# shamspias/fennec

Measured on AMD Instinct MI355X. Metric: megapixels/sec: 4K SSIMFast+GaussianBlur, higher is better.
Workload: dtype u8 (blur: exact int32 sums of 24-bit fixed-point weights on the i8 matrix pipe; fp64 SSIM)

## Files before the change

### fennec_amd/csrc/blur_mfma.hip

```cpp
#include <hip/hip_ext.h>

#include "common.hpp"
#include "devutil.hpp"

#include <algorithm>
#include <cmath>
#include <type_traits>
#include <vector>

namespace fnx {

typedef int v4i __attribute__((ext_vector_type(4)));

constexpr int MF_RMAX = 6;
constexpr int MF_P = 48;
constexpr int MF_WT = 64 * MF_P + 256;
constexpr int MF_SP = 352;
constexpr int MF_OP = 272;
constexpr int MF_SEG_SCORE = 272;
constexpr int MF_SEG_SCORE_WIDE = 544;

struct MfmaArgs {
    const uint8_t *src;
    const uint8_t *const *srcs;
    uint8_t *dst;
    uint8_t *const *dsts;
    int sstride, dstride, w, h;
    int tiles_x, tiles, seg;
    int radius;
    const uint32_t *tab;
    int seed_h, seed_v, thr;
    const int32_t *bx, *by;
    unsigned long long *slabs;
    int nbx, nby;
    int dbg;
};

__device__ __forceinline__ int mf_comb3(int hi, int mid, int lo)
{
    int t = hi * 256 + mid;
    asm volatile("" : "+v"(t));
    return t * 256 + lo;
}

__device__ __forceinline__ const double *mf_scalar_ptr(const double *p)
{
    const unsigned long long v = reinterpret_cast<unsigned long long>(p);
    const unsigned lo = __builtin_amdgcn_readfirstlane(static_cast<unsigned>(v)), hi = __builtin_amdgcn_readfirstlane(static_cast<unsigned>(v >> 32));
    return reinterpret_cast<const double *>((static_cast<unsigned long long>(hi) << 32) | lo);
}
typedef int mf_s16i __attribute__((ext_vector_type(16)));
__device__ __forceinline__ uint32_t mf_exact_u(const double *wd, const uint8_t *base, int step, int ring0, int mask)
{
    mf_s16i w0, w1;
    asm volatile("s_load_dwordx16 %0, %2, 0x0\n\ts_load_dwordx16 %1, %2, 0x40\n\ts_waitcnt lgkmcnt(0)" : "=&s"(w0), "=&s"(w1) : "s"(mf_scalar_ptr(wd)) : "memory");
    uint32_t v[13];
#pragma unroll
    for (int t = 0; t < 13; t++) v[t] = base[((ring0 + t) & mask) * step];
    double acc = 0;
#pragma unroll
    for (int t = 0; t < 13; t++) {
        const int lo = t < 8 ? w0[2 * (t & 7)] : w1[2 * (t & 7)], hi = t < 8 ? w0[2 * (t & 7) + 1] : w1[2 * (t & 7) + 1];
        acc = acc + u8_to_f64(v[t] ^ 0x80u) * __hiloint2double(hi, lo);
    }
    return clampF_dev(acc);
}

__device__ __forceinline__ void mf_box_add4(uint32_t *tbl, const u32x4 ro, uint32_t coln, const v4i cb)
{
#pragma unroll
    for (int k = 0; k < 4; k++)
        __hip_atomic_fetch_add(reinterpret_cast<uint32_t *>(reinterpret_cast<char *>(tbl) + ro[k] + coln), static_cast<uint32_t>(cb[k]),
                               __ATOMIC_RELAXED, __HIP_MEMORY_SCOPE_WORKGROUP);
}

template <bool SCORE, bool GUARD>
__global__ __launch_bounds__(256, GUARD ? 3 : 1) void blur_mfma_kernel(MfmaArgs a)
{
    constexpr int P = MF_P, WT = MF_WT, SP = MF_SP, OP = MF_OP;
    __shared__ __attribute__((aligned(16))) uint8_t s_t[4 * WT];
    __shared__ __attribute__((aligned(16))) uint8_t s_stage[2 * 16 * SP];
    __shared__ __attribute__((aligned(16))) uint8_t s_out[2 * 16 * OP];
    __shared__ __attribute__((aligned(16))) uint32_t s_rowh[SCORE ? MF_SEG_SCORE + 32 : 4];
    __shared__ __attribute__((aligned(16))) uint32_t s_rowv[SCORE ? MF_SEG_SCORE + 16 : 4];
    __shared__ uint32_t s_colbox[SCORE ? 64 : 1];
    extern __shared__ __attribute__((aligned(16))) uint32_t s_box[];

    const int tile = xcd_tile(blockIdx.x, a.tiles);
    if (tile < 0) return;
    const int z = blockIdx.y;
    const uint8_t *src = a.srcs ? a.srcs[z] : a.src;
    uint8_t *dst = a.dsts ? a.dsts[z] : a.dst;
    const int ty = tile / a.tiles_x, tx = tile - ty * a.tiles_x;
    const int x0 = tx * 64, y0 = ty * a.seg;
    const int tid = threadIdx.x, wave = tid >> 6, lane = tid & 63;
    const int r = lane & 15, g = lane >> 4;
    const int NJ = min(a.seg, ((a.h - y0 + 15) >> 4) << 4) >> 4;
    const int NI = NJ + 1;
    const bool xedge = x0 - 6 < 0 || x0 + 70 > a.w;

    const v4i *tbh = reinterpret_cast<const v4i *>(a.tab);
    const long *tbv = reinterpret_cast<const long *>(a.tab + 3 * 64 * 4);
    const v4i bh2 = tbh[lane], bh1 = tbh[64 + lane], bh0 = tbh[128 + lane];
    const long bv2 = tbv[lane], bv1 = tbv[64 + lane], bv0 = tbv[128 + lane];
    const bool alane = (r & 3) == 3;
    const int seed_hl = alane ? (1 << 23) + 128 : a.seed_h;
    const v4i sh = {seed_hl, seed_hl, seed_hl, seed_hl}, sv = {a.seed_v, a.seed_v, a.seed_v, a.seed_v};
    const v4i zero = {0, 0, 0, 0};
    const uint32_t sel01 = alane ? 0x0c0c0400u : 0x0c0c0703u, sel23 = alane ? 0x04000c0cu : 0x07030c0cu;

    uint8_t *tw = s_t + wave * WT;
    const int id1 = min(256 + tid, 16 * 19 - 1);
    const int srow0 = tid / 19, sch0 = tid - 19 * srow0, srow1 = id1 / 19, sch1 = id1 - 19 * srow1;
    const bool two = tid < 48;
    const int st_w0 = srow0 * SP + 16 * sch0, st_w1 = srow1 * SP + 16 * sch1;
    const int st_r = r * SP + 64 * wave + 16 * g;
    uint8_t *t_w = tw + r * P + 4 * g;
    const int m4 = r >> 2, mi = r & 3;
    const uint8_t *t_r = tw + (16 * m4 + mi) * P + 64 * m4 + 8 * g;
    const uint8_t *t_ro = tw + (16 * m4 + mi) * P + 64 * m4 + ((8 * g + 16) & 31);
    const uint8_t *t_ae = tw + (16 * g + 3) * P + 64 * g + r + 6;
    const uint8_t *t_ao = tw + (16 * g + 3) * P + 64 * g + ((r + 22) & 31);
    const int o_w = r * OP + 64 * wave + 16 * g;
    const int orow = tid >> 4, och = tid & 15;
    const int o_r = orow * OP + 16 * och;
    const int xo = x0 + 4 * och;

    v4i bbox = {0, 0, 0, 0}, sbox = {0, 0, 0, 0};
    uint32_t coln = 0;
    const int slabn = SCORE ? (a.nbx + 1) * (a.nby + 1) : 0;
    uint32_t *tbl_s = s_box, *tbl_b = s_box + 4 * slabn;
    auto score_setup = [&]() {
        if (!(a.dbg & 4)) for (int e = tid; e < 8 * slabn; e += 256) s_box[e] = 0;
        const int rowbytes = 16 * (a.nbx + 1);
        const int b0y = a.by[y0];
        for (int u = tid; u < 16 * NI; u += 256) {
            const int t = u - 6;
            const int v = (t >= 0 && t < a.seg && y0 + t < a.h) ? a.by[y0 + t] : -1;
            s_rowh[u] = rowbytes * ((v >= 0 && b0y >= 0) ? v - b0y : a.nby);
        }
        for (int t = tid; t < 16 * NJ; t += 256) {
            const int v = (t < a.seg && y0 + t < a.h) ? a.by[y0 + t] : -1;
            s_rowv[t] = rowbytes * ((v >= 0 && b0y >= 0) ? v - b0y : a.nby);
        }
        if (tid < 64) {
            const int b0x = a.bx[x0], v = x0 + tid < a.w ? a.bx[x0 + tid] : -1;
            s_colbox[tid] = (v >= 0 && b0x >= 0) ? v - b0x : 255u;
        }
        __syncthreads();
        uint32_t first = 255u;
        for (int i = 0; i < 16; i++) first = min(first, s_colbox[16 * wave + i]);
        const int slot = r / 3, ch = r - 3 * slot;
        int cnt = 0;
        for (int i = 0; i < 16; i++) cnt += (r < 15 && s_colbox[16 * wave + i] == first + slot) ? 1 : 0;
#pragma unroll
        for (int e = 0; e < 4; e++) {
            const bool in = r < 15 && first != 255u && s_colbox[16 * wave + 4 * g + e] == first + slot;
            bbox[e] = in ? (1 << (8 * ch)) : 0;
        }
        const int seed = 128 * cnt;
        sbox = (v4i){seed, seed, seed, seed};
        const uint32_t bc = (r < 15 && first != 255u && cnt > 0) ? first + slot : static_cast<uint32_t>(a.nbx);
        coln = 16u * bc + 4u * (r < 15 ? ch : 3);
    };

    const double *wd = reinterpret_cast<const double *>(a.tab + 3 * 64 * 4 + 3 * 64 * 2);

    auto stage_write = [&](const u32x4 (&d)[2], int buf) {
        uint8_t *sb = s_stage + buf * 16 * SP;
        *reinterpret_cast<u32x4 *>(sb + st_w0) = d[0] ^ 0x80808080u;
        if (two) *reinterpret_cast<u32x4 *>(sb + st_w1) = d[1] ^ 0x80808080u;
    };
    auto hset = [&](int s, int buf, int slot) {
        const uint8_t *sbuf = s_stage + buf * 16 * SP;
        const uint8_t *sb = sbuf + st_r;
        if constexpr (!GUARD && !SCORE) {
#pragma unroll
            for (int hf = 0; hf < 2; hf++) {
                v4i c2[2], c1[2], c0[2];
#pragma unroll
                for (int q2 = 0; q2 < 2; q2++) {
                    const v4i A = *reinterpret_cast<const v4i *>(sb + 16 * (2 * hf + q2));
                    c2[q2] = __builtin_amdgcn_mfma_i32_16x16x64_i8(A, bh2, zero, 0, 0, 0);
                    c1[q2] = __builtin_amdgcn_mfma_i32_16x16x64_i8(A, bh1, zero, 0, 0, 0);
                    c0[q2] = __builtin_amdgcn_mfma_i32_16x16x64_i8(A, bh0, sh, 0, 0, 0);
                }
#pragma unroll
                for (int q2 = 0; q2 < 2; q2++) {
                    const int qq = 2 * hf + q2;
                    v4i u;
#pragma unroll
                    for (int k = 0; k < 4; k++) u[k] = mf_comb3(c2[q2][k], c1[q2][k], c0[q2][k]);
                    const uint32_t t01 = __builtin_amdgcn_perm((uint32_t)u[1], (uint32_t)u[0], sel01);
                    const uint32_t t23 = __builtin_amdgcn_perm((uint32_t)u[3], (uint32_t)u[2], sel23);
                    *reinterpret_cast<uint32_t *>(t_w + (16 * qq) * P + 64 * qq + 16 * slot) = t01 | t23;
                }
                __builtin_amdgcn_sched_barrier(0);
            }
            return;
        }
        v4i c2[4], c1[4], c0[4];
#pragma unroll
        for (int qq = 0; qq < 4; qq++) {
            const v4i A = *reinterpret_cast<const v4i *>(sb + 16 * qq);
            c2[qq] = __builtin_amdgcn_mfma_i32_16x16x64_i8(A, bh2, zero, 0, 0, 0);
            c1[qq] = __builtin_amdgcn_mfma_i32_16x16x64_i8(A, bh1, zero, 0, 0, 0);
            c0[qq] = __builtin_amdgcn_mfma_i32_16x16x64_i8(A, bh0, sh, 0, 0, 0);
        }
        if constexpr (SCORE) {
            const u32x2 lo = *reinterpret_cast<const u32x2 *>(sb + 24), hi = *reinterpret_cast<const u32x2 *>(sb + 32);
            const v4i A = {(int)lo.x, (int)lo.y, (int)hi.x, (int)hi.y};
            const v4i cb = __builtin_amdgcn_mfma_i32_16x16x64_i8(A, bbox, sbox, 0, 0, 0);
            const u32x4 ro = *reinterpret_cast<const u32x4 *>(s_rowh + 16 * s + 4 * g);
            if (!(a.dbg & 1)) mf_box_add4(tbl_s, ro, coln, cb);
        }
        v4i u[4];
#pragma unroll
        for (int qq = 0; qq < 4; qq++)
#pragma unroll
            for (int k = 0; k < 4; k++) u[qq][k] = mf_comb3(c2[qq][k], c1[qq][k], c0[qq][k]);
#pragma unroll
        for (int qq = 0; qq < 4; qq++) {
            const uint32_t t01 = __builtin_amdgcn_perm((uint32_t)u[qq][1], (uint32_t)u[qq][0], sel01);
            const uint32_t t23 = __builtin_amdgcn_perm((uint32_t)u[qq][3], (uint32_t)u[qq][2], sel23);
            *reinterpret_cast<uint32_t *>(t_w + (16 * qq) * P + 64 * qq + 16 * slot) = t01 | t23;
        }
        if constexpr (GUARD) {
            uint32_t m[4];
#pragma unroll
            for (int qq = 0; qq < 4; qq++) {
                const uint32_t f0 = static_cast<uint32_t>(u[qq][0]) & 0x00ffffffu, f1 = static_cast<uint32_t>(u[qq][1]) & 0x00ffffffu;
                const uint32_t f2 = static_cast<uint32_t>(u[qq][2]) & 0x00ffffffu, f3 = static_cast<uint32_t>(u[qq][3]) & 0x00ffffffu;
                m[qq] = min(min(min(f0, f1), f2), f3);
            }
            const uint32_t mm = min(min(min(m[0], m[1]), m[2]), m[3]);
            if (__builtin_amdgcn_ballot_w64(mm < static_cast<uint32_t>(a.thr))) {
                uint32_t fl = 0;
#pragma unroll
                for (int qq = 0; qq < 4; qq++)
#pragma unroll
                    for (int k = 0; k < 4; k++) fl |= ((static_cast<uint32_t>(u[qq][k]) & 0x00ffffffu) < static_cast<uint32_t>(a.thr) ? 1u : 0u) << (4 * qq + k);
                unsigned long long todo = __builtin_amdgcn_ballot_w64(fl != 0);
                while (todo) {
                    const int L = __builtin_ctzll(todo);
                    todo &= todo - 1;
                    uint32_t flL = __builtin_amdgcn_readlane(fl, L);
                    const int rL = L & 15, gL = L >> 4;
                    while (flL) {
                        const int b = __builtin_ctz(flL), qq = b >> 2, k = b & 3;
                        flL &= flL - 1;
                        const uint32_t e = mf_exact_u(wd, sbuf + (4 * gL + k) * SP + 4 * (16 * wave + 4 * qq + (rL >> 2)) + (rL & 3), 4, 0, 0xffff) ^ 0x80u;
                        if (lane == L) *(t_w + (16 * qq) * P + 64 * qq + 16 * slot + k) = static_cast<uint8_t>(e);
                    }
                }
            }
        }
    };
    auto vset = [&](int j, int buf, auto oddt) {
        constexpr bool ODD = decltype(oddt)::value;
        long A[4];
        uint32_t al[4];
#pragma unroll
        for (int q = 0; q < 4; q++) A[q] = *reinterpret_cast<const long *>((ODD ? t_ro : t_r) + (4 * q) * P);
#pragma unroll
        for (int q = 0; q < 4; q++) al[q] = *((ODD ? t_ao : t_ae) + (4 * q) * P);
        int u[4][3];
        if constexpr (!GUARD && !SCORE) {
#pragma unroll
            for (int hf = 0; hf < 2; hf++) {
                v4i c2[2], c1[2], c0[2];
#pragma unroll
                for (int q2 = 0; q2 < 2; q2++) {
                    c2[q2] = __builtin_amdgcn_mfma_i32_16x16x32_i8(A[2 * hf + q2], bv2, zero, 0, 0, 0);
                    c1[q2] = __builtin_amdgcn_mfma_i32_16x16x32_i8(A[2 * hf + q2], bv1, zero, 0, 0, 0);
                    c0[q2] = __builtin_amdgcn_mfma_i32_16x16x32_i8(A[2 * hf + q2], bv0, sv, 0, 0, 0);
                }
#pragma unroll
                for (int q2 = 0; q2 < 2; q2++)
#pragma unroll
                    for (int i = 0; i < 3; i++) u[2 * hf + q2][i] = mf_comb3(c2[q2][i], c1[q2][i], c0[q2][i]);
                __builtin_amdgcn_sched_barrier(0);
            }
        } else {
            v4i c2[4], c1[4], c0[4];
#pragma unroll
            for (int q = 0; q < 4; q++) {
                c2[q] = __builtin_amdgcn_mfma_i32_16x16x32_i8(A[q], bv2, zero, 0, 0, 0);
                c1[q] = __builtin_amdgcn_mfma_i32_16x16x32_i8(A[q], bv1, zero, 0, 0, 0);
                c0[q] = __builtin_amdgcn_mfma_i32_16x16x32_i8(A[q], bv0, sv, 0, 0, 0);
            }
#pragma unroll
            for (int q = 0; q < 4; q++)
#pragma unroll
                for (int i = 0; i < 3; i++) u[q][i] = mf_comb3(c2[q][i], c1[q][i], c0[q][i]);
        }
        u32x4 o;
#pragma unroll
        for (int q = 0; q < 4; q++) {
            const uint32_t t01 = __builtin_amdgcn_perm((uint32_t)u[q][1], (uint32_t)u[q][0], 0x0c0c0703u);
            const uint32_t t23 = __builtin_amdgcn_perm(al[q], (uint32_t)u[q][2], 0x04030c0cu);
            o[q] = t01 | t23;
        }
        uint8_t *op = s_out + buf * 16 * OP + o_w;
        *reinterpret_cast<u32x4 *>(op) = o;
        if constexpr (GUARD) {
            uint32_t m[4];
#pragma unroll
            for (int q = 0; q < 4; q++)
                m[q] = min(min(static_cast<uint32_t>(u[q][0]) & 0x00ffffffu, static_cast<uint32_t>(u[q][1]) & 0x00ffffffu), static_cast<uint32_t>(u[q][2]) & 0x00ffffffu);
            const uint32_t mm = min(min(min(m[0], m[1]), m[2]), m[3]);
            if (__builtin_amdgcn_ballot_w64(mm < static_cast<uint32_t>(a.thr))) {
                uint32_t fl = 0;
#pragma unroll
                for (int q = 0; q < 4; q++)
#pragma unroll
                    for (int i = 0; i < 3; i++) fl |= ((static_cast<uint32_t>(u[q][i]) & 0x00ffffffu) < static_cast<uint32_t>(a.thr) ? 1u : 0u) << (4 * q + i);
                unsigned long long todo = __builtin_amdgcn_ballot_w64(fl != 0);
                while (todo) {
                    const int L = __builtin_ctzll(todo);
                    todo &= todo - 1;
                    uint32_t flL = __builtin_amdgcn_readlane(fl, L);
                    const int rL = L & 15, gL = L >> 4;
                    while (flL) {
                        const int b = __builtin_ctz(flL), q = b >> 2, i = b & 3;
                        flL &= flL - 1;
                        const uint32_t e = mf_exact_u(wd, tw + (16 * gL + 4 * q + i) * P + 64 * gL, 1, (ODD ? 16 : 0) + rL, 31);
                        if (lane == L) op[4 * q + i] = static_cast<uint8_t>(e);
                    }
                }
                if constexpr (SCORE) o = *reinterpret_cast<const u32x4 *>(op);
            }
        }
        if constexpr (SCORE) {
            const u32x4 os = o ^ 0x80808080u;
            const v4i A = {(int)os[0], (int)os[1], (int)os[2], (int)os[3]};
            const v4i cb = __builtin_amdgcn_mfma_i32_16x16x64_i8(A, bbox, sbox, 0, 0, 0);
            const u32x4 ro = *reinterpret_cast<const u32x4 *>(s_rowv + 16 * j + 4 * g);
            if (!(a.dbg & 1)) mf_box_add4(tbl_b, ro, coln, cb);
        }
    };

    auto march = [&](auto xedget) {
        constexpr bool XEDGE = decltype(xedget)::value;
        auto hload = [&](int i, u32x4 (&d)[2]) {
            const int ys = y0 - 6 + 16 * i;
            if constexpr (!XEDGE) {
                const uint8_t *sb = src + 4 * static_cast<ptrdiff_t>(x0 - 6);
                const int ya = clampi(ys + srow0, 0, a.h - 1), yb = clampi(ys + srow1, 0, a.h - 1);
                d[0] = *(g_u32x4 *)(sb + static_cast<ptrdiff_t>(ya) * a.sstride + 16 * sch0);
                d[1] = *(g_u32x4 *)(sb + static_cast<ptrdiff_t>(yb) * a.sstride + 16 * sch1);
            } else {
    #pragma unroll
                for (int k = 0; k < 2; k++) {
                    if (k == 1 && !two) break;
                    const int y = clampi(ys + (k ? srow1 : srow0), 0, a.h - 1);
                    const uint8_t *rowp = src + static_cast<size_t>(y) * a.sstride;
                    const int xc = x0 - 6 + 4 * (k ? sch1 : sch0);
    #pragma unroll
                    for (int e = 0; e < 4; e++) d[k][e] = ld_px(rowp, clampi(xc + e, 0, a.w - 1));
                }
            }
        };
        auto out_store = [&](int j, int buf) {
            const u32x4 o = *reinterpret_cast<const u32x4 *>(s_out + buf * 16 * OP + o_r);
            const int y = y0 + 16 * j + orow;
            if (y < a.h) {
                uint8_t *dp = dst + static_cast<size_t>(y) * a.dstride + 4 * static_cast<size_t>(xo);
                if (!XEDGE || xo + 3 < a.w) *(g_u32x4w *)(dp) = o;
                else {
    #pragma unroll
                    for (int e = 0; e < 4; e++) if (xo + e < a.w) *(g_u32w *)(dp + 4 * e) = o[e];
                }
            }
        };
        u32x4 ra[2], rb[2];
        hload(0, ra);
        __builtin_amdgcn_sched_barrier(0);
        hload(min(1, NI - 1), rb);
        __builtin_amdgcn_sched_barrier(0);
        if constexpr (SCORE) score_setup();
        auto step = [&](int s, u32x4 (&d)[2], auto oddv) {
            constexpr int par = decltype(oddv)::value ? 0 : 1;
            if (s < NI) stage_write(d, par);
            if (XEDGE) { if (s + 2 < NI) hload(s + 2, d); } else hload(min(s + 2, NI - 1), d);
            if (s >= 3 && s - 3 < NJ) out_store(s - 3, par);
            __syncthreads();
            if (s < NI) hset(s, par, par);
            if (s >= 1 && s - 1 < NJ) vset(s - 1, par, oddv);
        };
    #pragma unroll 1
        for (int s = 0; s < NJ + 3; s += 2) {
            step(s, ra, std::true_type{});
            step(s + 1, rb, std::false_type{});
        }

    };
    if (xedge) march(std::true_type{}); else march(std::false_type{});

    if (SCORE && !(a.dbg & 2)) {
        __syncthreads();
        unsigned long long *slab = a.slabs + (static_cast<size_t>(z) * a.tiles + tile) * 2 * slabn;
        for (int e = tid; e < 2 * slabn; e += 256) {
            const u32x4 v = *reinterpret_cast<const u32x4 *>(s_box + 4 * e);
            slab[e] = static_cast<unsigned long long>(v.x | (v.y << 16)) | (static_cast<unsigned long long>(v.z) << 32);
        }
    }
}

template <int NKH> struct MfWide {
    static constexpr int NKV = NKH <= 4 ? 1 : (NKH <= 7 ? 2 : 3);
    static constexpr int RFH = 8 * NKH - 2, RFV = 32 * NKV - 8;
    static constexpr int RF = RFH < RFV ? RFH : RFV;
    static constexpr int NC = 16 + RF / 2;
    static constexpr int NL = (16 * NC + 255) / 256;
    static constexpr int SP = 16 * NC + 48;
    static constexpr int NT = 2 * RF + 1;
    static constexpr int NS = 4 * NKV;
    static constexpr int RING = 16 * NS;
    static constexpr int P = RING + 16;
    static constexpr int WT = 64 * P + 256;
};

template <int NT>
__device__ __noinline__ uint32_t mf_exact_h_n(const uint8_t *p, const double *wd)
{
    double acc = 0;
#pragma unroll 15
    for (int t = 0; t < NT; t++) acc = acc + u8_to_f64(p[4 * t] ^ 0x80u) * wd[t];
    return clampF_dev(acc);
}
template <int NT, int RING = 64>
__device__ __noinline__ uint32_t mf_exact_v_n(const uint8_t *p, int ring0, const double *wd)
{
    double acc = 0;
#pragma unroll 15
    for (int t = 0; t < NT; t++) acc = acc + u8_to_f64(p[static_cast<unsigned>(ring0 + t) % static_cast<unsigned>(RING)] ^ 0x80u) * wd[t];
    return clampF_dev(acc);
}

template <int NT>
__device__ __forceinline__ uint32_t mf_exact_u_n(const double *wd, const uint8_t *base, int step, int ring0, int mask)
{
    double acc = 0;
#pragma unroll
    for (int t0 = 0; t0 < NT; t0 += 8) {
        mf_s16i w;
        asm volatile("s_load_dwordx16 %0, %1, %2\n\ts_waitcnt lgkmcnt(0)" : "=&s"(w) : "s"(mf_scalar_ptr(wd)), "n"(8 * t0) : "memory");
        uint32_t v[8];
#pragma unroll
        for (int t = 0; t < 8; t++) v[t] = base[((ring0 + t0 + min(t, NT - 1 - t0)) & mask) * step];
#pragma unroll
        for (int t = 0; t < 8; t++)
            if (t0 + t < NT) acc = acc + u8_to_f64(v[t] ^ 0x80u) * __hiloint2double(w[2 * t + 1], w[2 * t]);
    }
    return clampF_dev(acc);
}

template <int NKH, bool GUARD, bool SCORE = false>
__global__ __launch_bounds__(256, MfWide<NKH>::NKV == 3 ? 1 : 2) void blur_mfma_wide_kernel(MfmaArgs a)
{
    using C = MfWide<NKH>;
    constexpr int RF = C::RF, NC = C::NC, SP = C::SP, P = C::P, WT = C::WT, OP = MF_OP, NT = C::NT;
    constexpr int NKV = C::NKV, NS = C::NS, RING = C::RING, NL = C::NL;
    static_assert(!SCORE || (4 * RF) % 8 == 0, "the source-side A operand is read as two 8-byte halves");
    static_assert(!SCORE || NKV == 1, "the one-pass form is NKH = 2's");
    __shared__ __attribute__((aligned(16))) uint8_t s_t[4 * WT];
    __shared__ __attribute__((aligned(16))) uint8_t s_stage[2 * 16 * SP];
    __shared__ __attribute__((aligned(16))) uint8_t s_out[2 * 16 * OP];
    __shared__ __attribute__((aligned(16))) uint32_t s_rowh[SCORE ? MF_SEG_SCORE_WIDE + 48 : 4];
    __shared__ __attribute__((aligned(16))) uint32_t s_rowv[SCORE ? MF_SEG_SCORE_WIDE + 16 : 4];
    __shared__ uint32_t s_colbox[SCORE ? 64 : 1];
    extern __shared__ __attribute__((aligned(16))) uint32_t s_box[];

    const int tile = xcd_tile(blockIdx.x, a.tiles);
    if (tile < 0) return;
    const int z = blockIdx.y;
    const uint8_t *src = a.srcs ? a.srcs[z] : a.src;
    uint8_t *dst = a.dsts ? a.dsts[z] : a.dst;
    const int ty = tile / a.tiles_x, tx = tile - ty * a.tiles_x;
    const int x0 = tx * 64, y0 = ty * a.seg;
    const int tid = threadIdx.x, wave = tid >> 6, lane = tid & 63;
    const int r = lane & 15, g = lane >> 4;
    const int NJ = min(a.seg, ((a.h - y0 + 15) >> 4) << 4) >> 4;
    const int NI = NJ + NS - 1;
    const bool xedge = x0 - RF < 0 || x0 + 64 + RF > a.w;

    const v4i *tbh = reinterpret_cast<const v4i *>(a.tab);
    v4i bh[NKH][3];
#pragma unroll
    for (int kk = 0; kk < NKH; kk++)
#pragma unroll
        for (int l = 0; l < 3; l++) bh[kk][l] = tbh[(3 * kk + l) * 64 + lane];
    const v4i *tbv = tbh + 3 * NKH * 64;
    v4i bv[NKV][3];
#pragma unroll
    for (int c = 0; c < NKV; c++)
#pragma unroll
        for (int l = 0; l < 3; l++) bv[c][l] = tbv[(3 * c + l) * 64 + lane];
    const double *wd = reinterpret_cast<const double *>(tbv + 3 * NKV * 64);
    const bool alane = (r & 3) == 3;
    const int seed_hl = alane ? (1 << 23) + 128 : a.seed_h;
    const v4i sh = {seed_hl, seed_hl, seed_hl, seed_hl}, sv = {a.seed_v, a.seed_v, a.seed_v, a.seed_v};
    const v4i zero = {0, 0, 0, 0};
    const uint32_t sel01 = alane ? 0x0c0c0400u : 0x0c0c0703u, sel23 = alane ? 0x04000c0cu : 0x07030c0cu;

    uint8_t *tw = s_t + wave * WT;
    int srow[NL], sch[NL], st_w[NL];
    bool have[NL];
#pragma unroll
    for (int k = 0; k < NL; k++) {
        const int id = min(256 * k + tid, 16 * NC - 1);
        srow[k] = id / NC; sch[k] = id - NC * srow[k];
        st_w[k] = srow[k] * SP + 16 * sch[k];
        have[k] = 256 * k + tid < 16 * NC;
    }
    const int st_r = r * SP + 64 * wave + 16 * g;
    uint8_t *t_w = tw + r * P + 4 * g;
    const int m4 = r >> 2, mi = r & 3;
    const uint8_t *t_r = tw + (16 * m4 + mi) * P + 64 * m4;
    const uint8_t *t_a = tw + (16 * g + 3) * P + 64 * g;
    const int o_w = r * OP + 64 * wave + 16 * g;
    const int orow = tid >> 4, och = tid & 15;
    const int o_r = orow * OP + 16 * och;
    const int xo = x0 + 4 * och;

    v4i bbox = {0, 0, 0, 0}, sbox = {0, 0, 0, 0};
    uint32_t coln = 0;
    const int slabn = SCORE ? (a.nbx + 1) * (a.nby + 1) : 0;
    uint32_t *tbl_s = s_box, *tbl_b = s_box + 4 * slabn;
    auto score_setup = [&]() {
        for (int e = tid; e < 8 * slabn; e += 256) s_box[e] = 0;
        const int rowbytes = 16 * (a.nbx + 1);
        const int b0y = a.by[y0];
        for (int u = tid; u < 16 * NI; u += 256) {
            const int t = u - RF;
            const int v = (t >= 0 && t < a.seg && y0 + t < a.h) ? a.by[y0 + t] : -1;
            s_rowh[u] = rowbytes * ((v >= 0 && b0y >= 0) ? v - b0y : a.nby);
        }
        for (int t = tid; t < 16 * NJ; t += 256) {
            const int v = (t < a.seg && y0 + t < a.h) ? a.by[y0 + t] : -1;
            s_rowv[t] = rowbytes * ((v >= 0 && b0y >= 0) ? v - b0y : a.nby);
        }
        if (tid < 64) {
            const int b0x = a.bx[x0], v = x0 + tid < a.w ? a.bx[x0 + tid] : -1;
            s_colbox[tid] = (v >= 0 && b0x >= 0) ? v - b0x : 255u;
        }
        __syncthreads();
        uint32_t first = 255u;
        for (int i = 0; i < 16; i++) first = min(first, s_colbox[16 * wave + i]);
        const int slot = r / 3, ch = r - 3 * slot;
        int cnt = 0;
        for (int i = 0; i < 16; i++) cnt += (r < 15 && s_colbox[16 * wave + i] == first + slot) ? 1 : 0;
#pragma unroll
        for (int e = 0; e < 4; e++) {
            const bool in = r < 15 && first != 255u && s_colbox[16 * wave + 4 * g + e] == first + slot;
            bbox[e] = in ? (1 << (8 * ch)) : 0;
        }
        const int seed = 128 * cnt;
        sbox = (v4i){seed, seed, seed, seed};
        const uint32_t bc = (r < 15 && first != 255u && cnt > 0) ? first + slot : static_cast<uint32_t>(a.nbx);
        coln = 16u * bc + 4u * (r < 15 ? ch : 3);
    };

    auto stage_write = [&](const u32x4 (&d)[NL], int buf) {
        uint8_t *sb = s_stage + buf * 16 * SP;
        *reinterpret_cast<u32x4 *>(sb + st_w[0]) = d[0] ^ 0x80808080u;
#pragma unroll
        for (int k = 1; k < NL; k++)
            if (have[k]) *reinterpret_cast<u32x4 *>(sb + st_w[k]) = d[k] ^ 0x80808080u;
    };
    auto hset = [&](int s, int buf, int slot) {
        const uint8_t *sbuf = s_stage + buf * 16 * SP;
        const uint8_t *sb = sbuf + st_r;
        v4i c2[4], c1[4], c0[4];
#pragma unroll
        for (int qq = 0; qq < 4; qq++) { c2[qq] = zero; c1[qq] = zero; c0[qq] = sh; }
        if constexpr (SCORE) {
            const u32x2 lo = *reinterpret_cast<const u32x2 *>(sb + 4 * RF), hi = *reinterpret_cast<const u32x2 *>(sb + 4 * RF + 8);
            const v4i A = {(int)lo.x, (int)lo.y, (int)hi.x, (int)hi.y};
            const v4i cb = __builtin_amdgcn_mfma_i32_16x16x64_i8(A, bbox, sbox, 0, 0, 0);
            const u32x4 ro = *reinterpret_cast<const u32x4 *>(s_rowh + 16 * s + 4 * g);
#pragma unroll
            for (int k = 0; k < 4; k++)
                __hip_atomic_fetch_add(reinterpret_cast<uint32_t *>(reinterpret_cast<char *>(tbl_s) + ro[k] + coln), static_cast<uint32_t>(cb[k]),
                                       __ATOMIC_RELAXED, __HIP_MEMORY_SCOPE_WORKGROUP);
        }
#pragma unroll
        for (int kk = 0; kk < NKH; kk++)
#pragma unroll
            for (int qq = 0; qq < 4; qq++) {
                const v4i A = *reinterpret_cast<const v4i *>(sb + 16 * qq + 64 * kk);
                c2[qq] = __builtin_amdgcn_mfma_i32_16x16x64_i8(A, bh[kk][0], c2[qq], 0, 0, 0);
                c1[qq] = __builtin_amdgcn_mfma_i32_16x16x64_i8(A, bh[kk][1], c1[qq], 0, 0, 0);
                c0[qq] = __builtin_amdgcn_mfma_i32_16x16x64_i8(A, bh[kk][2], c0[qq], 0, 0, 0);
            }
        v4i u[4];
#pragma unroll
        for (int qq = 0; qq < 4; qq++)
#pragma unroll
            for (int k = 0; k < 4; k++) u[qq][k] = mf_comb3(c2[qq][k], c1[qq][k], c0[qq][k]);
#pragma unroll
        for (int qq = 0; qq < 4; qq++) {
            const uint32_t t01 = __builtin_amdgcn_perm((uint32_t)u[qq][1], (uint32_t)u[qq][0], sel01);
            const uint32_t t23 = __builtin_amdgcn_perm((uint32_t)u[qq][3], (uint32_t)u[qq][2], sel23);
            *reinterpret_cast<uint32_t *>(t_w + (16 * qq) * P + 64 * qq + 16 * slot) = t01 | t23;
        }
        if constexpr (GUARD) {
            uint32_t m[4];
#pragma unroll
            for (int qq = 0; qq < 4; qq++) {
                const uint32_t f0 = static_cast<uint32_t>(u[qq][0]) & 0x00ffffffu, f1 = static_cast<uint32_t>(u[qq][1]) & 0x00ffffffu;
                const uint32_t f2 = static_cast<uint32_t>(u[qq][2]) & 0x00ffffffu, f3 = static_cast<uint32_t>(u[qq][3]) & 0x00ffffffu;
                m[qq] = min(min(min(f0, f1), f2), f3);
            }
            const uint32_t mm = min(min(min(m[0], m[1]), m[2]), m[3]);
            if (__builtin_amdgcn_ballot_w64(mm < static_cast<uint32_t>(a.thr))) {
                uint32_t fl = 0;
#pragma unroll
                for (int qq = 0; qq < 4; qq++)
#pragma unroll
                    for (int k = 0; k < 4; k++) fl |= ((static_cast<uint32_t>(u[qq][k]) & 0x00ffffffu) < static_cast<uint32_t>(a.thr) ? 1u : 0u) << (4 * qq + k);
                if constexpr (NKH > 2) {
                    while (fl) {
                        const int b = __builtin_ctz(fl), qq = b >> 2, k = b & 3;
                        fl &= fl - 1;
                        const uint32_t e = mf_exact_h_n<NT>(sbuf + (4 * g + k) * SP + 4 * (16 * wave + 4 * qq + (r >> 2)) + (r & 3), wd) ^ 0x80u;
                        *(t_w + (16 * qq) * P + 64 * qq + 16 * slot + k) = static_cast<uint8_t>(e);
                    }
                }
                unsigned long long todo = NKH > 2 ? 0ull : __builtin_amdgcn_ballot_w64(fl != 0);
                while (todo) {
                    const int L = __builtin_ctzll(todo);
                    todo &= todo - 1;
                    uint32_t flL = __builtin_amdgcn_readlane(fl, L);
                    const int rL = L & 15, gL = L >> 4;
                    while (flL) {
                        const int b = __builtin_ctz(flL), qq = b >> 2, k = b & 3;
                        flL &= flL - 1;
                        const uint32_t e = mf_exact_u_n<NT>(wd, sbuf + (4 * gL + k) * SP + 4 * (16 * wave + 4 * qq + (rL >> 2)) + (rL & 3), 4, 0, 0xffff) ^ 0x80u;
                        if (lane == L) *(t_w + (16 * qq) * P + 64 * qq + 16 * slot + k) = static_cast<uint8_t>(e);
                    }
                }
            }
        }
    };
    auto vset = [&](int j, int buf) {
        uint32_t al[4];
        const int jm = static_cast<int>(static_cast<unsigned>(j) % static_cast<unsigned>(NS));
        const int ra_ = static_cast<int>(static_cast<unsigned>(16 * jm + r + RF) % static_cast<unsigned>(RING));
#pragma unroll
        for (int q = 0; q < 4; q++) al[q] = *(t_a + (4 * q) * P + ra_);
        v4i c2[4], c1[4], c0[4];
#pragma unroll
        for (int q = 0; q < 4; q++) { c2[q] = zero; c1[q] = zero; c0[q] = sv; }
#pragma unroll
        for (int c = 0; c < NKV; c++) {
            const int ro = 16 * static_cast<int>(static_cast<unsigned>(jm + 4 * c + g) % static_cast<unsigned>(NS));
            v4i A[4];
#pragma unroll
            for (int q = 0; q < 4; q++) A[q] = *reinterpret_cast<const v4i *>(t_r + (4 * q) * P + ro);
#pragma unroll
            for (int q = 0; q < 4; q++) {
                c2[q] = __builtin_amdgcn_mfma_i32_16x16x64_i8(A[q], bv[c][0], c2[q], 0, 0, 0);
                c1[q] = __builtin_amdgcn_mfma_i32_16x16x64_i8(A[q], bv[c][1], c1[q], 0, 0, 0);
                c0[q] = __builtin_amdgcn_mfma_i32_16x16x64_i8(A[q], bv[c][2], c0[q], 0, 0, 0);
            }
        }
        int u[4][3];
#pragma unroll
        for (int q = 0; q < 4; q++)
#pragma unroll
            for (int i = 0; i < 3; i++) u[q][i] = mf_comb3(c2[q][i], c1[q][i], c0[q][i]);
        u32x4 o;
#pragma unroll
        for (int q = 0; q < 4; q++) {
            const uint32_t t01 = __builtin_amdgcn_perm((uint32_t)u[q][1], (uint32_t)u[q][0], 0x0c0c0703u);
            const uint32_t t23 = __builtin_amdgcn_perm(al[q], (uint32_t)u[q][2], 0x04030c0cu);
            o[q] = t01 | t23;
        }
        uint8_t *op = s_out + buf * 16 * OP + o_w;
        *reinterpret_cast<u32x4 *>(op) = o;
        if constexpr (GUARD) {
            uint32_t m[4];
#pragma unroll
            for (int q = 0; q < 4; q++)
                m[q] = min(min(static_cast<uint32_t>(u[q][0]) & 0x00ffffffu, static_cast<uint32_t>(u[q][1]) & 0x00ffffffu), static_cast<uint32_t>(u[q][2]) & 0x00ffffffu);
            const uint32_t mm = min(min(min(m[0], m[1]), m[2]), m[3]);
            if (__builtin_amdgcn_ballot_w64(mm < static_cast<uint32_t>(a.thr))) {
                uint32_t fl = 0;
#pragma unroll
                for (int q = 0; q < 4; q++)
#pragma unroll
                    for (int i = 0; i < 3; i++) fl |= ((static_cast<uint32_t>(u[q][i]) & 0x00ffffffu) < static_cast<uint32_t>(a.thr) ? 1u : 0u) << (4 * q + i);
                if constexpr (NKH > 2) {
                    while (fl) {
                        const int b = __builtin_ctz(fl), q = b >> 2, i = b & 3;
                        fl &= fl - 1;
                        op[4 * q + i] = static_cast<uint8_t>(mf_exact_v_n<NT, RING>(tw + (16 * g + 4 * q + i) * P + 64 * g, 16 * jm + r, wd));
                    }
                }
                unsigned long long todo = NKH > 2 ? 0ull : __builtin_amdgcn_ballot_w64(fl != 0);
                while (todo) {
// ... 399 lines not shown
```

Before: 395,600.

## Software-pipeline MFMA chains and defer LDS box atomics in the SCORE blur path

In the SCORE variant, the horizontal and vertical MFMA passes are rewritten to interleave the next quad's MFMAs with the combine and pack ALU work of the current quad, using sched barriers to fix the order. The LDS atomic box-sum adds from the horizontal pass are deferred into the vertical pass so they overlap MFMA latency. Atomic addresses are precomputed as LDS offsets. The march loop is split into prologue, steady-state and epilogue phases so the steady phase drops its bounds checks, and the debug flags become compile-time zero outside develop builds. The risks are higher register pressure and rigid scheduling from the many sched barriers.

```diff
diff --git a/fennec_amd/csrc/blur_mfma.hip b/fennec_amd/csrc/blur_mfma.hip
--- a/fennec_amd/csrc/blur_mfma.hip
+++ b/fennec_amd/csrc/blur_mfma.hip
@@ -36,11 +36,15 @@
     int dbg;
 };
 
-__device__ __forceinline__ int mf_comb3(int hi, int mid, int lo)
+__device__ __forceinline__ int mf_comb_hi(int hi, int mid)
 {
     int t = hi * 256 + mid;
     asm volatile("" : "+v"(t));
-    return t * 256 + lo;
+    return t;
+}
+__device__ __forceinline__ int mf_comb3(int hi, int mid, int lo)
+{
+    return mf_comb_hi(hi, mid) * 256 + lo;
 }
 
 __device__ __forceinline__ const double *mf_scalar_ptr(const double *p)
@@ -66,12 +70,21 @@
     return clampF_dev(acc);
 }
 
-__device__ __forceinline__ void mf_box_add4(uint32_t *tbl, const u32x4 ro, uint32_t coln, const v4i cb)
+typedef __attribute__((address_space(3))) uint32_t mf_lds_u32;
+__device__ __forceinline__ void mf_box_addr4(uint32_t (&ad)[4], uint32_t *tbl, const u32x4 ro, uint32_t coln)
+{
+    const uint32_t base = static_cast<uint32_t>(reinterpret_cast<uintptr_t>((mf_lds_u32 *)tbl)) + coln;
+#pragma unroll
+    for (int k = 0; k < 4; k++) {
+        ad[k] = ro[k] + base;
+        asm volatile("" : "+v"(ad[k]));
+    }
+}
+__device__ __forceinline__ void mf_box_add4(const uint32_t (&ad)[4], const v4i cb)
 {
 #pragma unroll
     for (int k = 0; k < 4; k++)
-        __hip_atomic_fetch_add(reinterpret_cast<uint32_t *>(reinterpret_cast<char *>(tbl) + ro[k] + coln), static_cast<uint32_t>(cb[k]),
-                               __ATOMIC_RELAXED, __HIP_MEMORY_SCOPE_WORKGROUP);
+        __hip_atomic_fetch_add((mf_lds_u32 *)static_cast<uintptr_t>(ad[k]), static_cast<uint32_t>(cb[k]), __ATOMIC_RELAXED, __HIP_MEMORY_SCOPE_WORKGROUP);
 }
 
 template <bool SCORE, bool GUARD>
@@ -130,8 +143,13 @@
     uint32_t coln = 0;
     const int slabn = SCORE ? (a.nbx + 1) * (a.nby + 1) : 0;
     uint32_t *tbl_s = s_box, *tbl_b = s_box + 4 * slabn;
+#ifdef FNX_DEVELOP
+    const int dbg = a.dbg;
+#else
+    constexpr int dbg = 0;
+#endif
     auto score_setup = [&]() {
-        if (!(a.dbg & 4)) for (int e = tid; e < 8 * slabn; e += 256) s_box[e] = 0;
+        if (!(dbg & 4)) for (int e = tid; e < 8 * slabn; e += 256) s_box[e] = 0;
         const int rowbytes = 16 * (a.nbx + 1);
         const int b0y = a.by[y0];
         for (int u = tid; u < 16 * NI; u += 256) {
@@ -171,7 +189,10 @@
         *reinterpret_cast<u32x4 *>(sb + st_w0) = d[0] ^ 0x80808080u;
         if (two) *reinterpret_cast<u32x4 *>(sb + st_w1) = d[1] ^ 0x80808080u;
     };
-    auto hset = [&](int s, int buf, int slot) {
+    v4i h_cb = zero;
+    uint32_t h_ad[4] = {0, 0, 0, 0};
+    auto hset = [&](int s, int buf, int slot, auto defert) {
+        constexpr bool DEFER = decltype(defert)::value;
         const uint8_t *sbuf = s_stage + buf * 16 * SP;
         const uint8_t *sb = sbuf + st_r;
         if constexpr (!GUARD && !SCORE) {
@@ -199,31 +220,62 @@
             }
             return;
         }
-        v4i c2[4], c1[4], c0[4];
-#pragma unroll
-        for (int qq = 0; qq < 4; qq++) {
-            const v4i A = *reinterpret_cast<const v4i *>(sb + 16 * qq);
-            c2[qq] = __builtin_amdgcn_mfma_i32_16x16x64_i8(A, bh2, zero, 0, 0, 0);
-            c1[qq] = __builtin_amdgcn_mfma_i32_16x16x64_i8(A, bh1, zero, 0, 0, 0);
-            c0[qq] = __builtin_amdgcn_mfma_i32_16x16x64_i8(A, bh0, sh, 0, 0, 0);
-        }
+        v4i u[4];
         if constexpr (SCORE) {
+            __builtin_amdgcn_sched_barrier(0);
+            v4i A[4];
+#pragma unroll
+            for (int qq = 0; qq < 4; qq++) A[qq] = *reinterpret_cast<const v4i *>(sb + 16 * qq);
             const u32x2 lo = *reinterpret_cast<const u32x2 *>(sb + 24), hi = *reinterpret_cast<const u32x2 *>(sb + 32);
-            const v4i A = {(int)lo.x, (int)lo.y, (int)hi.x, (int)hi.y};
-            const v4i cb = __builtin_amdgcn_mfma_i32_16x16x64_i8(A, bbox, sbox, 0, 0, 0);
+            const v4i As = {(int)lo.x, (int)lo.y, (int)hi.x, (int)hi.y};
             const u32x4 ro = *reinterpret_cast<const u32x4 *>(s_rowh + 16 * s + 4 * g);
-            if (!(a.dbg & 1)) mf_box_add4(tbl_s, ro, coln, cb);
-        }
-        v4i u[4];
-#pragma unroll
-        for (int qq = 0; qq < 4; qq++)
-#pragma unroll
-            for (int k = 0; k < 4; k++) u[qq][k] = mf_comb3(c2[qq][k], c1[qq][k], c0[qq][k]);
-#pragma unroll
-        for (int qq = 0; qq < 4; qq++) {
-            const uint32_t t01 = __builtin_amdgcn_perm((uint32_t)u[qq][1], (uint32_t)u[qq][0], sel01);
-            const uint32_t t23 = __builtin_amdgcn_perm((uint32_t)u[qq][3], (uint32_t)u[qq][2], sel23);
-            *reinterpret_cast<uint32_t *>(t_w + (16 * qq) * P + 64 * qq + 16 * slot) = t01 | t23;
+            v4i c2 = __builtin_amdgcn_mfma_i32_16x16x64_i8(A[0], bh2, zero, 0, 0, 0);
+            v4i c1 = __builtin_amdgcn_mfma_i32_16x16x64_i8(A[0], bh1, zero, 0, 0, 0);
+            v4i c0 = __builtin_amdgcn_mfma_i32_16x16x64_i8(A[0], bh0, sh, 0, 0, 0);
+            __builtin_amdgcn_sched_barrier(0);
+            mf_box_addr4(h_ad, tbl_s, ro, coln);
+            __builtin_amdgcn_sched_barrier(0);
+#pragma unroll
+            for (int qq = 0; qq < 4; qq++) {
+                v4i n2 = zero, n1 = zero, n0 = zero;
+                if (qq < 3) n2 = __builtin_amdgcn_mfma_i32_16x16x64_i8(A[qq + 1], bh2, zero, 0, 0, 0);
+                else h_cb = __builtin_amdgcn_mfma_i32_16x16x64_i8(As, bbox, sbox, 0, 0, 0);
+                __builtin_amdgcn_sched_barrier(0);
+                int t[4];
+#pragma unroll
+                for (int k = 0; k < 4; k++) t[k] = mf_comb_hi(c2[k], c1[k]);
+                __builtin_amdgcn_sched_barrier(0);
+                if (qq < 3) { n1 = __builtin_amdgcn_mfma_i32_16x16x64_i8(A[qq + 1], bh1, zero, 0, 0, 0); __builtin_amdgcn_sched_barrier(0); }
+#pragma unroll
+                for (int k = 0; k < 4; k++) u[qq][k] = t[k] * 256 + c0[k];
+                __builtin_amdgcn_sched_barrier(0);
+                if (qq < 3) { n0 = __builtin_amdgcn_mfma_i32_16x16x64_i8(A[qq + 1], bh0, sh, 0, 0, 0); __builtin_amdgcn_sched_barrier(0); }
+                const uint32_t t01 = __builtin_amdgcn_perm((uint32_t)u[qq][1], (uint32_t)u[qq][0], sel01);
+                const uint32_t t23 = __builtin_amdgcn_perm((uint32_t)u[qq][3], (uint32_t)u[qq][2], sel23);
+                *reinterpret_cast<uint32_t *>(t_w + (16 * qq) * P + 64 * qq + 16 * slot) = t01 | t23;
+                __builtin_amdgcn_sched_barrier(0);
+                c2 = n2; c1 = n1; c0 = n0;
+            }
+            if constexpr (!DEFER) { if (!(dbg & 1)) mf_box_add4(h_ad, h_cb); }
+        } else {
+            v4i c2[4], c1[4], c0[4];
+#pragma unroll
+            for (int qq = 0; qq < 4; qq++) {
+                const v4i A = *reinterpret_cast<const v4i *>(sb + 16 * qq);
+                c2[qq] = __builtin_amdgcn_mfma_i32_16x16x64_i8(A, bh2, zero, 0, 0, 0);
+                c1[qq] = __builtin_amdgcn_mfma_i32_16x16x64_i8(A, bh1, zero, 0, 0, 0);
+                c0[qq] = __builtin_amdgcn_mfma_i32_16x16x64_i8(A, bh0, sh, 0, 0, 0);
+            }
+#pragma unroll
+            for (int qq = 0; qq < 4; qq++)
+#pragma unroll
+                for (int k = 0; k < 4; k++) u[qq][k] = mf_comb3(c2[qq][k], c1[qq][k], c0[qq][k]);
+#pragma unroll
+            for (int qq = 0; qq < 4; qq++) {
+                const uint32_t t01 = __builtin_amdgcn_perm((uint32_t)u[qq][1], (uint32_t)u[qq][0], sel01);
+                const uint32_t t23 = __builtin_amdgcn_perm((uint32_t)u[qq][3], (uint32_t)u[qq][2], sel23);
+                *reinterpret_cast<uint32_t *>(t_w + (16 * qq) * P + 64 * qq + 16 * slot) = t01 | t23;
+            }
         }
         if constexpr (GUARD) {
             uint32_t m[4];
@@ -256,8 +308,9 @@
             }
         }
     };
-    auto vset = [&](int j, int buf, auto oddt) {
+    auto vset = [&](int j, int buf, auto oddt, auto defert) {
         constexpr bool ODD = decltype(oddt)::value;
+        constexpr bool DEFER = decltype(defert)::value;
         long A[4];
         uint32_t al[4];
 #pragma unroll
@@ -265,6 +318,16 @@
 #pragma unroll
         for (int q = 0; q < 4; q++) al[q] = *((ODD ? t_ao : t_ae) + (4 * q) * P);
         int u[4][3];
+        u32x4 o;
+        u32x4 v_ro = {0, 0, 0, 0};
+        uint32_t v_ad[4] = {0, 0, 0, 0};
+        if constexpr (SCORE) v_ro = *reinterpret_cast<const u32x4 *>(s_rowv + 16 * j + 4 * g);
+        auto pack = [&](int q) {
+            const uint32_t t01 = __builtin_amdgcn_perm((uint32_t)u[q][1], (uint32_t)u[q][0], 0x0c0c0703u);
+            const uint32_t t23 = __builtin_amdgcn_perm(al[q], (uint32_t)u[q][2], 0x04030c0cu);
+            o[q] = t01 | t23;
+        };
+        if constexpr (SCORE) __builtin_amdgcn_sched_barrier(0);
         if constexpr (!GUARD && !SCORE) {
 #pragma unroll
             for (int hf = 0; hf < 2; hf++) {
@@ -281,6 +344,34 @@
                     for (int i = 0; i < 3; i++) u[2 * hf + q2][i] = mf_comb3(c2[q2][i], c1[q2][i], c0[q2][i]);
                 __builtin_amdgcn_sched_barrier(0);
             }
+        } else if constexpr (SCORE) {
+            v4i c2 = __builtin_amdgcn_mfma_i32_16x16x32_i8(A[0], bv2, zero, 0, 0, 0);
+            if constexpr (DEFER) { if (!(dbg & 1)) mf_box_add4(h_ad, h_cb); }
+            v4i c1 = __builtin_amdgcn_mfma_i32_16x16x32_i8(A[0], bv1, zero, 0, 0, 0);
+            v4i c0 = __builtin_amdgcn_mfma_i32_16x16x32_i8(A[0], bv0, sv, 0, 0, 0);
+            __builtin_amdgcn_sched_barrier(0);
+            mf_box_addr4(v_ad, tbl_b, v_ro, coln);
+            __builtin_amdgcn_sched_barrier(0);
+#pragma unroll
+            for (int q = 0; q < 4; q++) {
+                v4i n2 = zero, n1 = zero, n0 = zero;
+                if (q < 3) { n2 = __builtin_amdgcn_mfma_i32_16x16x32_i8(A[q + 1], bv2, zero, 0, 0, 0); __builtin_amdgcn_sched_barrier(0); }
+                int t[3];
+#pragma unroll
+                for (int i = 0; i < 3; i++) t[i] = mf_comb_hi(c2[i], c1[i]);
+                asm volatile("" : : "v"(c2), "v"(c1));
+                __builtin_amdgcn_sched_barrier(0);
+                if (q < 3) { n1 = __builtin_amdgcn_mfma_i32_16x16x32_i8(A[q + 1], bv1, zero, 0, 0, 0); __builtin_amdgcn_sched_barrier(0); }
+#pragma unroll
+                for (int i = 0; i < 3; i++) { u[q][i] = t[i] * 256 + c0[i]; asm volatile("" : "+v"(u[q][i])); }
+                asm volatile("" : : "v"(c0));
+                __builtin_amdgcn_sched_barrier(0);
+                if (q < 3) { n0 = __builtin_amdgcn_mfma_i32_16x16x32_i8(A[q + 1], bv0, sv, 0, 0, 0); __builtin_amdgcn_sched_barrier(0); }
+                pack(q);
+                asm volatile("" : "+v"(o[q]));
+                __builtin_amdgcn_sched_barrier(0);
+                c2 = n2; c1 = n1; c0 = n0;
+            }
         } else {
             v4i c2[4], c1[4], c0[4];
 #pragma unroll
@@ -294,15 +385,13 @@
 #pragma unroll
                 for (int i = 0; i < 3; i++) u[q][i] = mf_comb3(c2[q][i], c1[q][i], c0[q][i]);
         }
-        u32x4 o;
-#pragma unroll
-        for (int q = 0; q < 4; q++) {
-            const uint32_t t01 = __builtin_amdgcn_perm((uint32_t)u[q][1], (uint32_t)u[q][0], 0x0c0c0703u);
-            const uint32_t t23 = __builtin_amdgcn_perm(al[q], (uint32_t)u[q][2], 0x04030c0cu);
-            o[q] = t01 | t23;
+        if constexpr (!SCORE) {
+#pragma unroll
+            for (int q = 0; q < 4; q++) pack(q);
         }
         uint8_t *op = s_out + buf * 16 * OP + o_w;
         *reinterpret_cast<u32x4 *>(op) = o;
+        if constexpr (SCORE) __builtin_amdgcn_sched_barrier(0);
         if constexpr (GUARD) {
             uint32_t m[4];
 #pragma unroll
@@ -335,8 +424,7 @@
             const u32x4 os = o ^ 0x80808080u;
             const v4i A = {(int)os[0], (int)os[1], (int)os[2], (int)os[3]};
             const v4i cb = __builtin_amdgcn_mfma_i32_16x16x64_i8(A, bbox, sbox, 0, 0, 0);
-            const u32x4 ro = *reinterpret_cast<const u32x4 *>(s_rowv + 16 * j + 4 * g);
-            if (!(a.dbg & 1)) mf_box_add4(tbl_b, ro, coln, cb);
+            if (!(dbg & 1)) mf_box_add4(v_ad, cb);
         }
     };
 
@@ -379,25 +467,44 @@
         hload(min(1, NI - 1), rb);
         __builtin_amdgcn_sched_barrier(0);
         if constexpr (SCORE) score_setup();
-        auto step = [&](int s, u32x4 (&d)[2], auto oddv) {
+        auto step = [&](int s, u32x4 (&d)[2], auto oddv, auto steadyt) {
             constexpr int par = decltype(oddv)::value ? 0 : 1;
-            if (s < NI) stage_write(d, par);
-            if (XEDGE) { if (s + 2 < NI) hload(s + 2, d); } else hload(min(s + 2, NI - 1), d);
-            if (s >= 3 && s - 3 < NJ) out_store(s - 3, par);
+            constexpr bool STEADY = decltype(steadyt)::value;
+            if (STEADY || s < NI) stage_write(d, par);
+            if (XEDGE && !STEADY) { if (s + 2 < NI) hload(s + 2, d); } else hload(min(s + 2, NI - 1), d);
+            if (STEADY || (s >= 3 && s - 3 < NJ)) out_store(s - 3, par);
             __syncthreads();
-            if (s < NI) hset(s, par, par);
-            if (s >= 1 && s - 1 < NJ) vset(s - 1, par, oddv);
+            if (STEADY || s < NI) hset(s, par, par, std::bool_constant<SCORE && STEADY>{});
+            if (STEADY || (s >= 1 && s - 1 < NJ)) vset(s - 1, par, oddv, std::bool_constant<SCORE && STEADY>{});
         };
+        if constexpr (!SCORE) {
     #pragma unroll 1
-        for (int s = 0; s < NJ + 3; s += 2) {
-            step(s, ra, std::true_type{});
-            step(s + 1, rb, std::false_type{});
-        }
-
+            for (int s = 0; s < NJ + 3; s += 2) {
+                step(s, ra, std::true_type{}, std::false_type{});
+                step(s + 1, rb, std::false_type{}, std::false_type{});
+            }
+            return;
+        }
+        int s = 0;
+    #pragma unroll 1
+        for (; s < 4; s += 2) {
+            step(s, ra, std::true_type{}, std::false_type{});
+            step(s + 1, rb, std::false_type{}, std::false_type{});
+        }
+    #pragma unroll 1
+        for (; s + 1 <= NJ; s += 2) {
+            step(s, ra, std::true_type{}, std::true_type{});
+            step(s + 1, rb, std::false_type{}, std::true_type{});
+        }
+    #pragma unroll 1
+        for (; s < NJ + 3; s += 2) {
+            step(s, ra, std::true_type{}, std::false_type{});
+            step(s + 1, rb, std::false_type{}, std::false_type{});
+        }
     };
     if (xedge) march(std::true_type{}); else march(std::false_type{});
 
-    if (SCORE && !(a.dbg & 2)) {
+    if (SCORE && !(dbg & 2)) {
         __syncthreads();
         unsigned long long *slab = a.slabs + (static_cast<size_t>(z) * a.tiles + tile) * 2 * slabn;
         for (int e = tid; e < 2 * slabn; e += 256) {
```

Result: no change. 394,200 (-0.4%).
